# taaha-khan/2023-CompaCT-Image-Compression

Measured on AMD Instinct MI355X. Metric: MPixels/s encode+decode, 12-bit 512x512 CT batch, bytes-exact, higher is better.
Workload: dtype u16

## Files before the change

2023-compact-image-compression_amd/csrc/api.cpp:

```cpp
#include <dlfcn.h>
#include <unistd.h>
#include <zlib.h>

#include <atomic>
#include <chrono>
#include <condition_variable>
#include <functional>
#include <cstdarg>
#include <cstdio>
#include <cstdlib>
#include <cstring>
#include <map>
#include <mutex>
#include <string>
#include <thread>
#include <vector>

#include "../../include/compact_hip.h"
#include "cct_internal.h"
#include "host.h"
#include "handoff.h"

namespace cct {
bool gilbert_table(int width, int height, int32_t *out);
// ... 108 lines not shown
	}
	DecSlot(const DecSlot &) = delete;
	DecSlot &operator=(const DecSlot &) = delete;
};
constexpr int N_DEC_SLOTS = DEC_SLOTS;

struct Context {
	bool ready = false;
	pid_t pid = 0;
	int device = -1;
	hipStream_t stream = nullptr;
	int use_graph = 1;
	int deflate_fork = 1;
	int queue_ahead = 1;
	int decode_yields = 1;
	int compact_recs = 1;
	int enc_slots = 1;
	hipStream_t stream_dec = nullptr;
	std::map<std::pair<int, int>, ShapeTables> luts;
	int use_tiles = 1;
	int stream_tpg = STREAM_TPG;
	int last_path = -1;
	int runtime_bs = 0;
	int last_dec_path = -1;
	int dbg_skip = 0;
	int tuning_build = TUNING;
	int device_deflate = 1;
	int device_inflate = 1;
	int zlib_threads = 0;
	int wg_threads = 1024;
// ... 514 lines not shown
	int rc;
	void *base[DFL_REGIONS];
	for (int r = 0; r < DFL_REGIONS; r++) {
		if (dfl_region_needed(r, strategy) && (rc = E.z_ws[r].ensure(dfl_region_bytes(r, shape)))) return rc;
		base[r] = E.z_ws[r].p;
	}
	if ((rc = E.z_out.ensure((size_t)n * out_stride))) return rc;
	if ((rc = E.z_outsizes.ensure((size_t)n * 4))) return rc;
	const bool use_fork = g_ctx.deflate_fork != 0;
	if (use_fork && !E.stream_side) {
		const int crc = exclusive_section([&]() -> int { HIP_TRY(hipStreamCreateWithFlags(&E.stream_side, hipStreamNonBlocking)); return CCT_OK; });
		if (crc) return crc;
	}
	a.in = d_in; a.in_stride = in_stride; a.in_sizes = d_in_sizes;
	dfl_bind(a, base, shape);
	a.pos_mask = (g_ctx.compact_recs && mem_level == 8 && in_stride < ((size_t)1 << 22)) ? (1u << 22) - 1u : 0xFFFFFFFFu;
	const DevBuf &mr = E.z_ws[DFL_R_MATCH];
	if (dfl_uses_chains(strategy)) {
		if (E.z_mr_cleared != mr.p || E.z_mr_cleared_cap != mr.cap || E.z_gen_passes >= 16000u) {
			HIP_TRY(hipMemsetAsync(mr.p, 0, mr.cap, E.stream));
			HIP_TRY(hipMemsetAsync(E.z_ws[DFL_R_GEN].p, 0, 256, E.stream));
			E.z_mr_cleared = mr.p; E.z_mr_cleared_cap = mr.cap; E.z_gen_passes = 0;
		}
		E.z_gen_passes++;
	}
	a.out = (uint8_t *)E.z_out.p; a.out_stride = out_stride; a.out_sizes = (uint32_t *)E.z_outsizes.p;
	memcpy(a.header13, header13, 13);
	if (g_ctx.use_graph) {
		std::vector<uint8_t> key(sizeof(DeflateArgs) + 2 * sizeof(int));
		memcpy(key.data(), &a, sizeof(DeflateArgs));
// ... 1395 lines not shown
int rule_bool(int &v) { v = v ? 1 : 0; return CCT_OK; }
const Option OPTIONS[] = {
	{"zlib_threads", &Context::zlib_threads, [](int &v) { return v < 1 ? fail(CCT_E_ARG, "zlib_threads < 1") : CCT_OK; }},
	{"tile_path", &Context::use_tiles, [](int &v) {
		if (v == 3) return fail(CCT_E_ARG, "tile_path 3 (the four-kernel pipeline) has been removed");
		v = (v >= 0 && v <= 4) ? v : 1; return (int)CCT_OK; }},
	{"stream_tpg", &Context::stream_tpg, [](int &v) { v = (v == 1 || v == 2 || v == 4) ? v : STREAM_TPG; return (int)CCT_OK; }},
	{"runtime_block_size", &Context::runtime_bs, rule_bool},
	{"device_deflate", &Context::device_deflate, rule_bool},
	{"device_inflate", &Context::device_inflate, rule_bool},
	{"deflate_graph", &Context::use_graph, rule_bool},
	{"deflate_compact_records", &Context::compact_recs, rule_bool},
	{"decode_yields", &Context::decode_yields, rule_bool},
	{"queue_ahead", &Context::queue_ahead, rule_bool},
	{"deflate_fork", &Context::deflate_fork, rule_bool},
	{"encode_slots", &Context::enc_slots, [](int &v) { v = std::max(1, std::min(v, N_ENC_SLOTS)); return (int)CCT_OK; }},
	{"decode_slots", &Context::dec_slots, [](int &v) { v = std::max(1, std::min(v, N_DEC_SLOTS)); return (int)CCT_OK; }},
	{"inflate_lanes", &Context::inflate_lanes, [](int &v) {
		return v != 0 && v != 256 && v != 512 ? fail(CCT_E_ARG, "inflate_lanes must be 0 (automatic), 256 or 512") : CCT_OK; }},
	{"png_unfilter_waves", &Context::png_unfilter_waves, [](int &v) {
		return v != 1 && v != 2 && v != 4 && v != 8 ? fail(CCT_E_ARG, "png_unfilter_waves must be 1, 2, 4 or 8") : CCT_OK; }},
	{"wg_threads", &Context::wg_threads, [](int &v) {
		return v != 256 && v != 512 && v != 1024 ? fail(CCT_E_ARG, "wg_threads must be 256, 512 or 1024") : CCT_OK; }},
	{"last_encode_path", &Context::last_path, nullptr, true},
	{"last_decode_path", &Context::last_dec_path, nullptr, true},
	{"last_inflate_lanes", &Context::last_inflate_lanes, nullptr, true},
	{"debug_skip", &Context::dbg_skip, rule_any, false, true},
	{"tuning_build", &Context::tuning_build, nullptr, true, true},
};
const Option *find_option(const char *key)
// ... 31 lines not shown
```

2023-compact-image-compression_amd/csrc/deflate_kernels.hip:

```cpp
#include <hip/hip_runtime.h>
#include <cstring>
#include <algorithm>

#include "cct_internal.h"
#include "wave_device.h"
#include "../../include/compact_hip.h"

namespace cct {
namespace {

constexpr int MIN_MATCH = 3, MAX_MATCH = 258, WSIZE = 32768;
constexpr int MIN_LOOKAHEAD = MAX_MATCH + MIN_MATCH + 1;
constexpr int MAX_DIST = WSIZE - MIN_LOOKAHEAD;
constexpr int TOO_FAR = 4096;
constexpr int BLOCK_SYMS = 16383;
constexpr int BLOCK_SYMS_ML9 = 32767;
constexpr int L_CODES = 286, D_CODES = 30, BL_CODES = 19, HEAP_SIZE = 2 * L_CODES + 1;
constexpr int END_BLOCK = 256, MAX_BITS = 15, MAX_BL_BITS = 7;
constexpr uint32_t Z_FILTERED = 1, Z_HUFFMAN_ONLY = 2, Z_RLE = 3, Z_FIXED = 4;
__host__ __device__ __forceinline__ bool short_pass(uint32_t strategy) { return strategy == Z_HUFFMAN_ONLY || strategy == Z_RLE; }

__constant__ uint8_t c_extra_lbits[29] = {0,0,0,0,0,0,0,0,1,1,1,1,2,2,2,2,3,3,3,3,4,4,4,4,5,5,5,5,0};
__constant__ uint8_t c_extra_dbits[30] = {0,0,0,0,1,1,2,2,3,3,4,4,5,5,6,6,7,7,8,8,9,9,10,10,11,11,12,12,13,13};
__constant__ uint8_t c_extra_blbits[19] = {0,0,0,0,0,0,0,0,0,0,0,0,0,0,0,0,2,3,7};
// ... 988 lines not shown
	alignas(16) uint32_t heap[HEAP_SIZE + 11];
	uint32_t bl_count[MAX_BITS + 1];
	uint16_t next_code[MAX_BITS + 1];
	int heap_len, heap_max, max_code, overflow, lmax, dmax;
	uint32_t opt_len, static_len, dyn_body_bits;
	uint32_t hdr_bits[160];
	uint32_t hdr_nbits;
	int ntok, btype, max_blindex;
	uint8_t extra_l[29], extra_d[30], extra_bl[19], bl_order[19];
	__device__ __forceinline__ uint32_t *hist_l() { return heap; }
	__device__ __forceinline__ uint32_t *hist_d() { return heap + L_CODES + 2; }
	__device__ __forceinline__ uint8_t *length_code() { return reinterpret_cast<uint8_t *>(dad); }
	__device__ __forceinline__ uint8_t *dist_code() { return reinterpret_cast<uint8_t *>(dad) + 256; }
	__device__ __forceinline__ uint16_t *tok() { return dad; }
};
static_assert(sizeof(TreeScratch) <= 8192, "13 tree waves per CU: keep the working set around 8 KB");
static_assert(HEAP_SIZE >= L_CODES + D_CODES, "token list fits dad[]");
static_assert((HEAP_SIZE + 1) * 4 >= (L_CODES + 2 + D_CODES) * 4 && HEAP_SIZE * 2 >= 768, "aliases fit");
__device__ __forceinline__ uint32_t static_llen(int n) { return n <= 143 ? 8u : n <= 255 ? 9u : n <= 279 ? 7u : 8u; }

typedef __attribute__((address_space(3))) uint16_t lds_u16;
struct TreeView { lds_u16 *freq, *dad, *len, *code; };

__device__ __forceinline__ void pqdownheap(TreeScratch &S, int k, int hl)
{
	const uint32_t v = S.heap[k];
	for (int j = k << 1; j <= hl; j = k << 1) {
		const uint2 pr = *reinterpret_cast<const uint2 *>(&S.heap[j]);
		const int right = (j < hl && pr.y <= (pr.x | 1023u)) ? 1 : 0;
		const uint32_t e = right ? pr.y : pr.x;
		if (v <= (e | 1023u)) break;
// ... 2 lines not shown
	}
	S.heap[k] = v;
}

__device__ __forceinline__ TreeView view_of(TreeScratch &S, int kind)
{
	if (kind == 0) return TreeView{(lds_u16 *)S.freq, (lds_u16 *)S.dad, (lds_u16 *)S.len, (lds_u16 *)S.code};
	if (kind == 1) return TreeView{(lds_u16 *)S.dfreq, (lds_u16 *)S.ddad, (lds_u16 *)S.dlen, (lds_u16 *)S.dcode};
	return TreeView{(lds_u16 *)S.bfreq, (lds_u16 *)S.bdad, (lds_u16 *)S.blen, (lds_u16 *)S.bcode};
}
__device__ __forceinline__ int elems_of(int kind) { return kind == 0 ? L_CODES : kind == 1 ? D_CODES : BL_CODES; }

__device__ void tree_leaves(TreeScratch &S, int kind)
{
	const TreeView t = view_of(S, kind);
	const int lane = threadIdx.x, elems = elems_of(kind);
	const uint64_t lt_mask = (1ull << lane) - 1ull;
	int max_code = -1;
	uint32_t nleaf = 0;
	for (int n0 = 0; n0 < elems; n0 += 64) {
		const int n = n0 + lane;
		const uint32_t f = n < elems ? t.freq[n] : 0u;
		const uint64_t bal = __ballot(f != 0);
		if (f != 0) S.heap[1 + nleaf + (uint32_t)__popcll(bal & lt_mask)] = (f << 15) | (uint32_t)n;
		else if (n < elems) t.len[n] = 0;
		if (bal) max_code = n0 + 63 - __clzll((long long)bal);
		nleaf += (uint32_t)__popcll(bal);
	}
	if (lane == 0) { S.heap_len = (int)nleaf; S.max_code = max_code; }
}

constexpr int TREE_SIFTS = 8;
__device__ void tree_heap(TreeScratch &S, int kind)
{
	const TreeView t = view_of(S, kind);
	const int lane = threadIdx.x;
	int max_code = S.max_code, h = S.heap_len;
	while (h < 2) {
		const int node = max_code < 2 ? ++max_code : 0;
		h++;
		if (lane == 0) {
			t.freq[node] = 1; S.opt_len--;
			S.heap[h] = (1u << 15) | (uint32_t)node;
			if (kind == 0) S.static_len -= static_llen(node);
			else if (kind == 1) S.static_len -= 5;
		}
	}
	__syncthreads();
	for (int d = 31 - __clz(h >> 1); d >= 0; d--) {
		const int lo = 1 << d, hi = min((2 << d) - 1, h >> 1);
		for (int n0 = lo; n0 <= hi; n0 += 64) {
			if (n0 + lane <= hi) pqdownheap(S, n0 + lane, h);
			__builtin_amdgcn_wave_barrier();
		}
	}
	if (lane < TREE_SIFTS) {
		uint32_t v = 0, k = 1, hl = 0, w = 0;
		bool moving = false;
		const uint32_t sink = HEAP_SIZE + 3 + lane;
		auto tick = [&]() {
			const uint32_t j = k << 1;
			const uint2 pr = *reinterpret_cast<const uint2 *>(&S.heap[j]);
			const uint32_t right = (j < hl && pr.y <= (pr.x | 1023u)) ? 1u : 0u;
// ... 38 lines not shown
			if (h < 2) break;
			tick();
		}
		while (__ballot(moving)) tick();
		if (lane == 0) {
			S.heap[--hm] = en;
			S.heap_len = h; S.heap_max = hm;
			S.max_code = max_code;
		}
	}
}

__device__ void tree_depths(TreeScratch &S, int kind)
{
	const TreeView t = view_of(S, kind);
	const int lane = threadIdx.x;
	const int max_length = kind == 2 ? MAX_BL_BITS : MAX_BITS;
	const int base = kind == 0 ? 257 : 0;
	const int max_code = S.max_code, heap_max = S.heap_max;
	const uint32_t root = S.heap[heap_max];
	constexpr uint16_t UNKNOWN = 0xFFFF;
	for (int h = heap_max + 1 + lane; h < HEAP_SIZE; h += 64) t.len[S.heap[h] & 1023u] = UNKNOWN;
	if (lane == 0) t.len[root & 1023u] = 0;
	if (lane <= MAX_BITS) S.bl_count[lane] = 0;
	__syncthreads();
	for (bool again = true; again;) {
		again = false;
		for (int h0 = heap_max + 1; h0 < HEAP_SIZE; h0 += 64) {
			const int h = h0 + lane;
			bool unknown = false;
			if (h < HEAP_SIZE) {
				const int n = (int)(S.heap[h] & 1023u);
				if (t.len[n] == UNKNOWN) {
					const uint32_t ld = t.len[t.dad[n]];
					if (ld == UNKNOWN) unknown = true;
					else t.len[n] = (uint16_t)min(ld + 1u, (uint32_t)max_length);
				}
			}
			if (__ballot(unknown)) again = true;
		}
		__syncthreads();
	}
	int overflow = 0;
	for (int h0 = heap_max + 1; h0 < HEAP_SIZE; h0 += 64) {
		const int h = h0 + lane;
		const bool clamped = h < HEAP_SIZE && t.len[t.dad[S.heap[h] & 1023u]] == (uint32_t)max_length;
		overflow += (int)__popcll(__ballot(clamped));
	}
	uint32_t o = 0, st = 0;
	for (int n = lane; n <= max_code; n += 64) {
		const uint32_t f = t.freq[n];
		if (f == 0) continue;
		const uint32_t bits = t.len[n];
		atomicAdd(&S.bl_count[bits], 1u);
		uint32_t xbits = 0;
		if (n >= base) xbits = kind == 0 ? S.extra_l[n - base] : kind == 1 ? S.extra_d[n] : S.extra_bl[n];
// ... 27 lines not shown
				if ((uint32_t)t.len[m] != (uint32_t)bits) {
					S.opt_len += ((uint32_t)bits - t.len[m]) * t.freq[m];
					t.len[m] = (uint16_t)bits;
				}
				n--;
			}
		}
	}
	uint32_t code = 0;
	for (int bits = 1; bits <= MAX_BITS; bits++) { code = (code + S.bl_count[bits - 1]) << 1; S.next_code[bits] = (uint16_t)code; }
}

__device__ void tree_codes(TreeScratch &S, int kind)
{
	const TreeView t = view_of(S, kind);
	const int lane = threadIdx.x, max_code = S.max_code;
	const uint64_t lt_mask = (1ull << lane) - 1ull;
	uint32_t seen[MAX_BITS + 1];
#pragma unroll
	for (int b = 1; b <= MAX_BITS; b++) seen[b] = S.next_code[b];
	for (int n0 = 0; n0 <= max_code; n0 += 64) {
		const int n = n0 + lane;
		const int len = n <= max_code ? (int)t.len[n] : 0;
		uint32_t mine = 0;
#pragma unroll
		for (int b = 1; b <= MAX_BITS; b++) {
			const uint64_t bal = __ballot(len == b);
			if (len == b) mine = seen[b] + (uint32_t)__popcll(bal & lt_mask);
			seen[b] += (uint32_t)__popcll(bal);
		}
		if (len != 0) t.code[n] = (uint16_t)(__brev(mine) >> (32 - len));
	}
}

__device__ void scan_tree_wave(TreeScratch &S, const TreeView &t, int max_code)
{
	const int lane = threadIdx.x;
	constexpr int NCH = (L_CODES + 63) / 64;
	const int n_el = max_code + 1;
	uint32_t v[NCH];
	uint64_t startmask[NCH];
#pragma unroll
	for (int c = 0; c < NCH; c++) {
		const int n = c * 64 + lane;
		v[c] = n < n_el ? (uint32_t)t.len[n] : 0xFFFFu;
		const uint32_t before = n == 0 ? 0xFFFFFFFFu : (uint32_t)t.len[max(n - 1, 0)];
		startmask[c] = __ballot(n < n_el && v[c] != before);
	}
	uint16_t *tk = S.tok();
	uint32_t base = (uint32_t)S.ntok;
#pragma unroll
	for (int c = 0; c < NCH; c++) {
// ... 47 lines not shown
		}
		base += chunk_tok;
	}
	if (lane == 0) S.ntok = (int)base;
}

__device__ __forceinline__ void hdr_or(TreeScratch &S, uint32_t pos, uint32_t value, uint32_t n)
{
	const uint32_t w = pos >> 5, sh = pos & 31u;
	atomicOr(&S.hdr_bits[w], value << sh);
	if (sh + n > 32u) atomicOr(&S.hdr_bits[w + 1], value >> (32u - sh));
}

__device__ void send_header(TreeScratch &S)
{
	const int lane = threadIdx.x;
	const int nbl = S.max_blindex + 1;
	if (lane == 0) hdr_or(S, 0, (uint32_t)(S.lmax + 1 - 257) | ((uint32_t)(S.dmax + 1 - 1) << 5) | ((uint32_t)(nbl - 4) << 10), 14);
	if (lane < nbl) hdr_or(S, 14u + 3u * (uint32_t)lane, S.blen[S.bl_order[lane]], 3);
	uint32_t base = 14u + 3u * (uint32_t)nbl;
	const uint16_t *tk = S.tok();
	const int nt = S.ntok;
	for (int c0 = 0; c0 < nt; c0 += 64) {
		const int i = c0 + lane;
		uint32_t nbits = 0, val = 0;
		if (i < nt) {
			const uint32_t sym = tk[i] & 31u, ex = tk[i] >> 5;
			const uint32_t cl = S.blen[sym];
			nbits = cl + S.extra_bl[sym];
			val = (uint32_t)S.bcode[sym] | (ex << cl);
		}
		uint32_t chunk_bits;
		const uint32_t ex = wave_excl_scan(nbits, chunk_bits);
		if (nbits) hdr_or(S, base + ex, val, nbits);
		base += chunk_bits;
	}
	if (lane == 0) S.hdr_nbits = base;
}

constexpr int TREE_BLOCKS = 1;

__device__ __forceinline__ uint32_t window_base(uint32_t top, uint32_t L, uint32_t strategy)
{
	const uint32_t lam = strategy == Z_HUFFMAN_ONLY ? 0u : strategy == Z_RLE ? (uint32_t)MAX_MATCH : (uint32_t)MIN_LOOKAHEAD - 1u;
	const uint32_t kf = L >= 65536u ? (L - 65536u) / 32768u + 1u : 0u;
	uint32_t k = 0;
	if (top >= 65536u - lam) k = min((top - (65536u - lam)) / 32768u + 1u, kf);
	if (k == kf && 32768u * k + (uint32_t)(WSIZE + MAX_DIST) <= top && L <= top + lam) k++;
	return 32768u * k;
}
__global__ void __launch_bounds__(64) dfl_tree_kernel(DeflateArgs a)
{
	__shared__ TreeScratch S4[TREE_BLOCKS];
	const int s = blockIdx.y, m0 = blockIdx.x * TREE_BLOCKS, lane = threadIdx.x;
	const uint32_t T = a.total_syms[s];
	const uint32_t L = a.in_sizes[s];
	const uint32_t BS = a.block_syms;
	uint32_t nfull = T / BS;
	if (T % BS == 0 && nfull > 0 && !short_pass(a.strategy) && a.postloop_lit[s]) nfull--;
	const uint32_t nblocks = nfull + 1;
	BlockMeta *meta = a.block_meta + (size_t)s * a.max_blocks;
	if ((uint32_t)m0 >= nblocks) return;
	const int nb = (int)min((uint32_t)TREE_BLOCKS, nblocks - (uint32_t)m0);
	const uint32_t *bend = a.blk_end + (size_t)s * a.max_blocks;
	const bool owner = lane < nb;
#ifdef CCT_TREE_PROF
	long long tp[16]; int tpi = 0;
#define TREE_STAMP() do { if (tpi < 16) tp[tpi++] = clock64(); } while (0)
#else
#define TREE_STAMP() do {} while (0)
#endif
	TREE_STAMP();

	for (int q = 0; q < nb; q++) {
		TreeScratch &S = S4[q];
		const int m = m0 + q;
		const bool last = (uint32_t)m == nblocks - 1;
		const uint32_t first = (uint32_t)m * BS;
		const uint32_t nsym = last ? T - first : BS;
		const uint32_t *sym = a.sym + (size_t)s * a.in_stride + first;
		for (int i = lane; i < HEAP_SIZE; i += 64) { S.freq[i] = 0; S.len[i] = 0; }
		for (int i = lane; i < L_CODES + 2; i += 64) S.code[i] = 0;
		for (int i = lane; i < 2 * D_CODES + 1; i += 64) { S.dfreq[i] = 0; S.dlen[i] = 0; S.ddad[i] = 0; }
		for (int i = lane; i < D_CODES + 2; i += 64) S.dcode[i] = 0;
		for (int i = lane; i < 2 * BL_CODES + 1; i += 64) { S.bfreq[i] = 0; S.blen[i] = 0; S.bdad[i] = 0; }
		for (int i = lane; i < BL_CODES + 1; i += 64) S.bcode[i] = 0;
		uint8_t *length_code = S.length_code(), *dist_code = S.dist_code();
		{
			uint8_t dc[8], lc4[4];
#pragma unroll
			for (int k = 0; k < 8; k++) dc[k] = c_dist_code[lane + 64 * k];
#pragma unroll
			for (int k = 0; k < 4; k++) lc4[k] = c_length_code[lane + 64 * k];
			const int l29 = min(lane, 28), l30 = min(lane, 29), l19 = min(lane, 18);
			const uint8_t xl = c_extra_lbits[l29], xd = c_extra_dbits[l30], xb = c_extra_blbits[l19], bo = c_bl_order[l19];
#pragma unroll
			for (int k = 0; k < 8; k++) dist_code[lane + 64 * k] = dc[k];
#pragma unroll
			for (int k = 0; k < 4; k++) length_code[lane + 64 * k] = lc4[k];
			if (lane < 29) S.extra_l[lane] = xl;
			if (lane < 30) S.extra_d[lane] = xd;
			if (lane < 19) { S.extra_bl[lane] = xb; S.bl_order[lane] = bo; }
		}
		uint32_t *hl = S.hist_l(), *hd = S.hist_d();
		for (int i = lane; i < L_CODES; i += 64) hl[i] = 0;
		if (lane < D_CODES) hd[lane] = 0;
		__syncthreads();
		{
			const uint32_t lasts = nsym ? nsym - 1 : 0;
			uint32_t nv[16];
#pragma unroll
			for (int k = 0; k < 16; k++) nv[k] = sym[min((uint32_t)(k * 64 + lane), lasts)];
			for (uint32_t i0 = 0; i0 < nsym; i0 += 64 * 16) {
				uint32_t v[16];
#pragma unroll
				for (int k = 0; k < 16; k++) v[k] = nv[k];
#pragma unroll
				for (int k = 0; k < 16; k++) nv[k] = sym[min(i0 + 1024u + (uint32_t)(k * 64 + lane), lasts)];
#pragma unroll
				for (int k = 0; k < 16; k++) {
					if (i0 + (uint32_t)(k * 64 + lane) >= nsym) continue;
					const uint32_t dist = v[k] >> 16, lc = v[k] & 0xFFu;
					if (dist == 0) atomicAdd(&hl[lc], 1u);
					else {
						const uint32_t d1 = dist - 1;
						atomicAdd(&hl[length_code[lc] + 256 + 1], 1u);
						atomicAdd(&hd[d1 < 256 ? dist_code[d1] : dist_code[256 + (d1 >> 7)]], 1u);
					}
				}
			}
		}
		__syncthreads();
		for (int i = lane; i < L_CODES; i += 64) S.freq[i] = (uint16_t)hl[i];
		if (lane < D_CODES) S.dfreq[lane] = (uint16_t)hd[lane];
		for (int i = lane; i < 160; i += 64) S.hdr_bits[i] = 0;
		if (lane == 0) { S.opt_len = 0; S.static_len = 0; S.hdr_nbits = 0; S.ntok = 0; S.btype = 0; S.max_blindex = 0; }
		__syncthreads();
		if (lane == 0) S.freq[END_BLOCK] = 1;
		for (int i = lane; i < HEAP_SIZE; i += 64) S.dad[i] = 0;
	}
	__syncthreads();
	TREE_STAMP();
#pragma unroll 1
	for (int kind = 0; kind < 3; kind++) {
		if (kind == 2) {
			if (owner) S4[lane].dyn_body_bits = S4[lane].opt_len;
			__syncthreads();
			for (int q = 0; q < nb; q++) {
				TreeScratch &S = S4[q];
				scan_tree_wave(S, view_of(S, 0), S.lmax);
				__syncthreads();
				scan_tree_wave(S, view_of(S, 1), S.dmax);
				__syncthreads();
				if (lane < BL_CODES) { S.bfreq[lane] = (uint16_t)S.hdr_bits[lane]; S.hdr_bits[lane] = 0; }
			}
			__syncthreads();
		}
		for (int q = 0; q < nb; q++) tree_leaves(S4[q], kind);
		__syncthreads();
		TREE_STAMP();
		for (int q = 0; q < nb; q++) tree_heap(S4[q], kind);
		__syncthreads();
		TREE_STAMP();
		for (int q = 0; q < nb; q++) tree_depths(S4[q], kind);
		__syncthreads();
		if (owner) {
			tree_fix(S4[lane], kind);
			if (kind == 0) S4[lane].lmax = S4[lane].max_code; else if (kind == 1) S4[lane].dmax = S4[lane].max_code;
		}
		__syncthreads();
		for (int q = 0; q < nb; q++) tree_codes(S4[q], kind);
		__syncthreads();
		TREE_STAMP();
	}
	if (owner) {
		TreeScratch &S = S4[lane];
		const int m = m0 + lane;
		const bool last = (uint32_t)m == nblocks - 1;
		const uint32_t first = (uint32_t)m * BS;
		const uint32_t nsym = last ? T - first : BS;
		const uint32_t in_begin = m == 0 ? 0u : bend[m - 1];
		const uint32_t in_end = last ? L : bend[m];
		int max_blindex;
		for (max_blindex = BL_CODES - 1; max_blindex >= 3; max_blindex--)
			if (S.blen[S.bl_order[max_blindex]] != 0) break;
		S.opt_len += 3 * ((uint32_t)max_blindex + 1) + 5 + 5 + 4;
		uint32_t opt_lenb = (S.opt_len + 3 + 7) >> 3;
		const uint32_t static_lenb = (S.static_len + 3 + 7) >> 3;
		if (static_lenb <= opt_lenb) opt_lenb = static_lenb;
		const uint32_t stored_len = in_end - in_begin;
		const bool in_window = in_begin >= window_base(last ? L : a.blk_top[(size_t)s * a.max_blocks + m], L, a.strategy);
		BlockMeta bm;
		bm.in_begin = in_begin; bm.stored_len = stored_len; bm.first_sym = first; bm.nsym = nsym; bm.last = last ? 1u : 0u;
		if (in_window && stored_len + 4 <= opt_lenb) {
			bm.type = 0; bm.hdr_nbits = 0; bm.body_bits = 0;
		} else if (a.strategy == Z_FIXED || static_lenb == opt_lenb) {
			bm.type = 1; bm.hdr_nbits = 0; bm.body_bits = S.static_len;
		} else {
			bm.type = 2; bm.hdr_nbits = 0;
			bm.body_bits = S.dyn_body_bits;
		}
		S.btype = (int)bm.type; S.max_blindex = max_blindex;
		meta[m] = bm;
		if (m == 0) a.n_blocks[s] = nblocks;
	}
	__syncthreads();
	for (int q = 0; q < nb; q++) {
		TreeScratch &S = S4[q];
		if (S.btype != 2) continue;
		send_header(S);
		__syncthreads();
		BlockTables *bt = a.block_tables + ((size_t)s * a.max_blocks + m0 + q);
		for (int i = lane; i * 32 < (int)S.hdr_nbits; i += 64) bt->hdr_bits[i] = S.hdr_bits[i];
		if (lane == 0) meta[m0 + q].hdr_nbits = S.hdr_nbits;
	}
	__syncthreads();
	TREE_STAMP();
#ifdef CCT_TREE_PROF
	if (s == 0 && m0 == 0 && lane == 0) {
		printf("[tree prof] nb=%d:", nb);
		for (int i = 1; i < tpi; i++) printf(" %lld", tp[i] - tp[i - 1]);
		printf("  (hist | leaves0 heap0 rest0 | scan+leaves1 heap1 rest1 | scan_tree+leaves2 heap2 rest2 | final)\n");
	}
#endif
	for (int q = 0; q < nb; q++) {
		TreeScratch &S = S4[q];
		BlockTables *bt = a.block_tables + ((size_t)s * a.max_blocks + m0 + q);
		for (int i = lane; i < L_CODES; i += 64) { bt->lcode[i] = S.code[i]; bt->llen[i] = (uint8_t)S.len[i]; }
		if (lane < D_CODES) { bt->dcode[lane] = S.dcode[lane]; bt->dlen[lane] = (uint8_t)S.dlen[lane]; }
	}
}

__global__ void __launch_bounds__(256) dfl_adler_kernel(DeflateArgs a)
{
	__shared__ unsigned long long sa[256], sb[256];
	const int s = blockIdx.x;
	const uint32_t L = a.in_sizes[s];
	const uint8_t *in = a.in + (size_t)s * a.in_stride;
	unsigned long long A = 0, B = 0;
	const uint32_t nfull = L / 16;
	constexpr int U = 8;
	for (uint32_t g0 = threadIdx.x; g0 < nfull; g0 += blockDim.x * U) {
		uint4 v[U];
#pragma unroll
		for (int u = 0; u < U; u++) v[u] = *reinterpret_cast<const uint4 *>(in + (size_t)min(g0 + (uint32_t)u * blockDim.x, nfull - 1) * 16);
// ... 317 lines not shown
		return true;
	}
	if (!deflate_level_args(level, a)) return false;
	if (strategy == (int)Z_FIXED) a.zlib_flg = 0x01;
	return true;
}

bool deflate_mem_level_args(int mem_level, DeflateArgs &a)
{
	if (mem_level != 8 && mem_level != 9) return false;
	a.hash_bits = (uint32_t)mem_level + 7u;
	a.block_syms = (1u << (mem_level + 6)) - 1u;
	return true;
}

hipError_t deflate_init_tables()
{
	uint8_t length_code[256]; uint16_t base_length[29]; uint8_t dist_code[512]; uint16_t base_dist[30];
	uint16_t static_lcode[288]; uint8_t static_llen[288]; uint16_t static_dcode[30];
	static const int xl[29] = {0,0,0,0,0,0,0,0,1,1,1,1,2,2,2,2,3,3,3,3,4,4,4,4,5,5,5,5,0};
	static const int xd[30] = {0,0,0,0,1,1,2,2,3,3,4,4,5,5,6,6,7,7,8,8,9,9,10,10,11,11,12,12,13,13};
	int length = 0, code, n, dist = 0;
	for (code = 0; code < 28; code++) {
		base_length[code] = (uint16_t)length;
		for (n = 0; n < (1 << xl[code]); n++) length_code[length++] = (uint8_t)code;
	}
	length_code[length - 1] = (uint8_t)code;
	base_length[28] = 0;
	for (code = 0; code < 16; code++) {
		base_dist[code] = (uint16_t)dist;
// ... 11 lines not shown
	while (n <= 279) { static_llen[n++] = 7; bl_count[7]++; }
	while (n <= 287) { static_llen[n++] = 8; bl_count[8]++; }
	unsigned c = 0;
	for (int bits = 1; bits <= 15; bits++) { c = (c + bl_count[bits - 1]) << 1; next_code[bits] = (uint16_t)c; }
	auto rev = [](unsigned v, int len) { unsigned r = 0; do { r |= v & 1; v >>= 1; r <<= 1; } while (--len > 0); return r >> 1; };
	for (n = 0; n < 288; n++) static_lcode[n] = (uint16_t)rev(next_code[static_llen[n]]++, static_llen[n]);
	for (n = 0; n < 30; n++) static_dcode[n] = (uint16_t)rev((unsigned)n, 5);
	hipError_t e;
	if ((e = hipMemcpyToSymbol(HIP_SYMBOL(c_length_code), length_code, sizeof length_code)) != hipSuccess) return e;
	if ((e = hipMemcpyToSymbol(HIP_SYMBOL(c_base_length), base_length, sizeof base_length)) != hipSuccess) return e;
	if ((e = hipMemcpyToSymbol(HIP_SYMBOL(c_dist_code), dist_code, sizeof dist_code)) != hipSuccess) return e;
	if ((e = hipMemcpyToSymbol(HIP_SYMBOL(c_base_dist), base_dist, sizeof base_dist)) != hipSuccess) return e;
	if ((e = hipMemcpyToSymbol(HIP_SYMBOL(c_static_lcode), static_lcode, sizeof static_lcode)) != hipSuccess) return e;
	if ((e = hipMemcpyToSymbol(HIP_SYMBOL(c_static_llen), static_llen, sizeof static_llen)) != hipSuccess) return e;
	if ((e = hipMemcpyToSymbol(HIP_SYMBOL(c_static_dcode), static_dcode, sizeof static_dcode)) != hipSuccess) return e;
	return hipSuccess;
}

static hipError_t launch_deflate_short(const DeflateArgs &a, int n, hipStream_t st)
{
	const bool ml9 = a.block_syms == (uint32_t)BLOCK_SYMS_ML9;
	const int gx = (int)std::min<size_t>(64, (a.in_stride + 255) / 256);
	launch_clear(a, n, st);
	if (a.strategy == Z_RLE) {
		hipLaunchKernelGGL((dfl_run_len_kernel<false, 15>), dim3(gx, n), dim3(256), 0, st, a);
		hipLaunchKernelGGL(dfl_rle_rec_kernel, dim3(gx, n), dim3(256), 0, st, a);
		hipLaunchKernelGGL(dfl_offsets2_kernel, dim3(256), dim3(256), 0, st, a, n);
		hipLaunchKernelGGL(dfl_walk_kernel, dim3(n), dim3(WALK_T), 0, st, a, n);
		if (ml9) hipLaunchKernelGGL(dfl_symbols_kernel<BLOCK_SYMS_ML9>, dim3(gx, n), dim3(256), 0, st, a);
		else hipLaunchKernelGGL(dfl_symbols_kernel<BLOCK_SYMS>, dim3(gx, n), dim3(256), 0, st, a);
	} else {
		if (ml9) hipLaunchKernelGGL(dfl_huff_symbols_kernel<BLOCK_SYMS_ML9>, dim3(gx, n), dim3(256), 0, st, a);
		else hipLaunchKernelGGL(dfl_huff_symbols_kernel<BLOCK_SYMS>, dim3(gx, n), dim3(256), 0, st, a);
	}
	hipLaunchKernelGGL(dfl_adler_kernel, dim3(n), dim3(256), 0, st, a);
	hipLaunchKernelGGL(dfl_tree_kernel, dim3((a.max_blocks + TREE_BLOCKS - 1) / TREE_BLOCKS, n), dim3(64), 0, st, a);
	hipLaunchKernelGGL(dfl_layout_kernel, dim3(n), dim3(64), 0, st, a, n);
	hipLaunchKernelGGL(dfl_emit_kernel, dim3(a.max_blocks, n), dim3(256), 0, st, a);
	return hipGetLastError();
}

hipError_t launch_deflate(const DeflateArgs &a, int n, hipStream_t st, hipStream_t side, const hipEvent_t *ev)
{
	hipError_t e;
	const bool ml9 = a.hash_bits == 16;
	if ((a.hash_bits != 15 && !ml9) || a.block_syms != (uint32_t)(ml9 ? BLOCK_SYMS_ML9 : BLOCK_SYMS)) return hipErrorInvalidValue;
	if (ml9 && a.pos_mask != 0xFFFFFFFFu) return hipErrorInvalidValue;
	if ((a.out_stride & 3) || ((uintptr_t)a.out & 3)) return hipErrorInvalidValue;
	if (short_pass(a.strategy)) return launch_deflate_short(a, n, st);
	hipLaunchKernelGGL(dfl_offsets_kernel, dim3(64), dim3(256), 0, st, a, n);
	const int gx = (int)std::min<size_t>(64, (a.in_stride + 255) / 256);
	if (ml9) {
		hipLaunchKernelGGL((dfl_run_len_kernel<true, 16>), dim3(gx, n), dim3(256), 0, st, a);
		hipLaunchKernelGGL((dfl_sort_pass_kernel<true, 16>), dim3(n), dim3(1024), 0, st, a);
		hipLaunchKernelGGL((dfl_sort_pass_kernel<false, 16>), dim3(n), dim3(1024), 0, st, a);
	} else {
		hipLaunchKernelGGL((dfl_run_len_kernel<true, 15>), dim3(gx, n), dim3(256), 0, st, a);
		hipLaunchKernelGGL((dfl_sort_pass_kernel<true, 15>), dim3(n), dim3(1024), 0, st, a);
		hipLaunchKernelGGL((dfl_sort_pass_kernel<false, 15>), dim3(n), dim3(1024), 0, st, a);
	}
	const bool fork = side != nullptr && ev != nullptr;
	hipStream_t s2 = fork ? side : st;
	if (fork) {
// ... 21 lines not shown
		if ((e = hipEventRecord(ev[2], s2)) != hipSuccess) return e;
		if ((e = hipStreamWaitEvent(s2, ev[1], 0)) != hipSuccess) return e;
		if ((e = hipStreamWaitEvent(st, ev[2], 0)) != hipSuccess) return e;
	}
	hipLaunchKernelGGL(dfl_match_heavy_kernel, dim3(gx, n8), dim3(256), 0, s2, a, n);
	hipLaunchKernelGGL(dfl_adler_kernel, dim3(n), dim3(256), 0, s2, a);
	hipLaunchKernelGGL(dfl_match_run_kernel, dim3(gx, n8), dim3(256), 0, st, a, n);
	if (fork) {
		if ((e = hipEventRecord(ev[3], s2)) != hipSuccess) return e;
		if ((e = hipStreamWaitEvent(st, ev[3], 0)) != hipSuccess) return e;
	}
	hipLaunchKernelGGL(dfl_rec_kernel, dim3(gx, n), dim3(256), 0, st, a);
	hipLaunchKernelGGL(dfl_walk_kernel, dim3(n), dim3(WALK_T), 0, st, a, n);
	if (ml9) hipLaunchKernelGGL(dfl_symbols_kernel<BLOCK_SYMS_ML9>, dim3(gx, n), dim3(256), 0, st, a);
	else hipLaunchKernelGGL(dfl_symbols_kernel<BLOCK_SYMS>, dim3(gx, n), dim3(256), 0, st, a);
	hipLaunchKernelGGL(dfl_tree_kernel, dim3((a.max_blocks + TREE_BLOCKS - 1) / TREE_BLOCKS, n), dim3(64), 0, st, a);
	hipLaunchKernelGGL(dfl_layout_kernel, dim3(n), dim3(64), 0, st, a, n);
	hipLaunchKernelGGL(dfl_emit_kernel, dim3(a.max_blocks, n), dim3(256), 0, st, a);
	return hipGetLastError();
}

__global__ void __launch_bounds__(256) dfl_pack_exact_kernel(const uint8_t *src, size_t stride, const uint32_t *sizes,
                                                             const uint64_t *offsets, uint8_t *dst)
{
	const int s = blockIdx.y;
	const uint32_t nbytes = sizes[s];
	const uint8_t *in = src + (size_t)s * stride;
	uint8_t *out = dst + offsets[s];
	const uint32_t head = min((uint32_t)(-(uintptr_t)out & 3u), nbytes);
	const uint32_t nd = (nbytes - head) >> 2;
	const uint32_t tid = blockIdx.x * blockDim.x + threadIdx.x, nth = gridDim.x * blockDim.x;
// ... 23 lines not shown
```

2023-compact-image-compression_amd/csrc/deflate_workspace.h:

```cpp
#pragma once
#include <stddef.h>
#include <stdint.h>

#if defined(__HIPCC__)
#include <hip/hip_runtime.h>
#define DFL_HD __host__ __device__ __forceinline__
#else
#define DFL_HD inline
#endif

namespace cct {

struct BlockMeta {
	uint64_t bit_off;
	uint32_t type;
	uint32_t last;
	uint32_t first_sym, nsym;
	uint32_t in_begin, stored_len;
	uint32_t hdr_nbits, body_bits;
};
struct BlockTables {
	uint16_t lcode[286]; uint8_t llen[286];
	uint16_t dcode[30]; uint8_t dlen[30];
	uint32_t hdr_bits[160];
// ... 9 lines not shown
	uint32_t *run_counts; int run_chunks;
	uint32_t *sort_hist;
	uint16_t *run_len;
	uint32_t *rec32, *exit_pos, *exit_cnt;
	uint32_t *blk_entry, *blk_symbase;
	uint32_t *total_syms, *postloop_lit, *n_blocks, *adler, *heavy_count, *deep_count, *run_end_count;
	uint32_t *blk_end;
	uint32_t *blk_top;
	BlockMeta *block_meta; BlockTables *block_tables;
	int max_blocks;
	uint8_t *out; size_t out_stride; uint32_t *out_sizes;
	uint8_t header13[16];
	uint32_t good, max_lazy, nice, max_chain, zlib_flg;
	uint32_t strategy, min_len;
	uint32_t hash_bits, block_syms;
};

constexpr int SORT_HIST = 512;
constexpr int RUNLEN_OUT = 2048 - 264;
constexpr int BLK_ENTRY_GRAIN = 64;
enum DflCounter { DFL_SEG_BEGIN, DFL_SEG_END, DFL_TOTAL_SYMS, DFL_POSTLOOP_LIT, DFL_N_BLOCKS, DFL_ADLER, DFL_HEAVY_COUNT,
                  DFL_DEEP_COUNT, DFL_RUN_END_COUNT, DFL_COUNTERS };

DFL_HD int dfl_run_chunks(size_t in_stride) { return (int)(in_stride / RUNLEN_OUT + 1); }
DFL_HD int dfl_max_blocks(size_t in_stride, uint32_t block_syms) { return (int)(in_stride / block_syms + 2); }
DFL_HD size_t dfl_blk_words(size_t in_stride) { return in_stride / BLK_ENTRY_GRAIN; }
DFL_HD size_t dfl_hist_words(size_t n, size_t run_chunks) { return n * (SORT_HIST + 2 * run_chunks); }

DFL_HD size_t zlib_bound(size_t n, bool mem_level_8)
{
// ... 85 lines not shown
```

Baseline: 17960.

## Pack sixteen Huffman tree waves per workgroup with device-side launch selection

The deflate tree kernel now runs one deflate block per wavefront and can pack 16 waves per workgroup, each with its own LDS TreeScratch. Workgroup barriers become wavefront-scoped fences and barriers. In automatic mode both the 16-wave and 1-wave variants are launched, and each decides on the device, from the total workgroup count versus the CU count, whether it should do the work. This is meant to spread tree building across more CUs and raise occupancy, at the cost of an extra kernel launch and a per-wave scan over all slices' block counts.

```diff
diff --git a/2023-compact-image-compression_amd/csrc/api.cpp b/2023-compact-image-compression_amd/csrc/api.cpp
--- a/2023-compact-image-compression_amd/csrc/api.cpp
+++ b/2023-compact-image-compression_amd/csrc/api.cpp
@@ -146,6 +146,7 @@
 	int deflate_fork = 1;
 	int queue_ahead = 1;
 	int decode_yields = 1;
+	int tree_waves = 0;
 	int compact_recs = 1;
 	int enc_slots = 1;
 	hipStream_t stream_dec = nullptr;
@@ -690,6 +691,7 @@
 	}
 	a.in = d_in; a.in_stride = in_stride; a.in_sizes = d_in_sizes;
 	dfl_bind(a, base, shape);
+	a.tree_waves = (uint32_t)g_ctx.tree_waves;
 	a.pos_mask = (g_ctx.compact_recs && mem_level == 8 && in_stride < ((size_t)1 << 22)) ? (1u << 22) - 1u : 0xFFFFFFFFu;
 	const DevBuf &mr = E.z_ws[DFL_R_MATCH];
 	if (dfl_uses_chains(strategy)) {
@@ -2115,6 +2117,8 @@
 	{"decode_yields", &Context::decode_yields, rule_bool},
 	{"queue_ahead", &Context::queue_ahead, rule_bool},
 	{"deflate_fork", &Context::deflate_fork, rule_bool},
+	{"tree_waves", &Context::tree_waves, [](int &v) {
+		return v != 0 && v != 1 && v != 16 ? fail(CCT_E_ARG, "tree_waves must be 0 (automatic), 1 or 16") : CCT_OK; }},
 	{"encode_slots", &Context::enc_slots, [](int &v) { v = std::max(1, std::min(v, N_ENC_SLOTS)); return (int)CCT_OK; }},
 	{"decode_slots", &Context::dec_slots, [](int &v) { v = std::max(1, std::min(v, N_DEC_SLOTS)); return (int)CCT_OK; }},
 	{"inflate_lanes", &Context::inflate_lanes, [](int &v) {
diff --git a/2023-compact-image-compression_amd/csrc/deflate_kernels.hip b/2023-compact-image-compression_amd/csrc/deflate_kernels.hip
--- a/2023-compact-image-compression_amd/csrc/deflate_kernels.hip
+++ b/2023-compact-image-compression_amd/csrc/deflate_kernels.hip
@@ -1026,7 +1026,12 @@
 	__device__ __forceinline__ uint8_t *dist_code() { return reinterpret_cast<uint8_t *>(dad) + 256; }
 	__device__ __forceinline__ uint16_t *tok() { return dad; }
 };
-static_assert(sizeof(TreeScratch) <= 8192, "13 tree waves per CU: keep the working set around 8 KB");
+static_assert(16 * sizeof(TreeScratch) <= 160 * 1024, "a workgroup of 16 tree waves has to fit the LDS of a CU");
+__device__ __forceinline__ void tree_wave_sync()
+{
+	__builtin_amdgcn_fence(__ATOMIC_ACQ_REL, "wavefront");
+	__builtin_amdgcn_wave_barrier();
+}
 static_assert(HEAP_SIZE >= L_CODES + D_CODES, "token list fits dad[]");
 static_assert((HEAP_SIZE + 1) * 4 >= (L_CODES + 2 + D_CODES) * 4 && HEAP_SIZE * 2 >= 768, "aliases fit");
 __device__ __forceinline__ uint32_t static_llen(int n) { return n <= 143 ? 8u : n <= 255 ? 9u : n <= 279 ? 7u : 8u; }
@@ -1059,7 +1064,7 @@
 __device__ void tree_leaves(TreeScratch &S, int kind)
 {
 	const TreeView t = view_of(S, kind);
-	const int lane = threadIdx.x, elems = elems_of(kind);
+	const int lane = threadIdx.x & 63, elems = elems_of(kind);
 	const uint64_t lt_mask = (1ull << lane) - 1ull;
 	int max_code = -1;
 	uint32_t nleaf = 0;
@@ -1079,7 +1084,7 @@
 __device__ void tree_heap(TreeScratch &S, int kind)
 {
 	const TreeView t = view_of(S, kind);
-	const int lane = threadIdx.x;
+	const int lane = threadIdx.x & 63;
 	int max_code = S.max_code, h = S.heap_len;
 	while (h < 2) {
 		const int node = max_code < 2 ? ++max_code : 0;
@@ -1091,7 +1096,7 @@
 			else if (kind == 1) S.static_len -= 5;
 		}
 	}
-	__syncthreads();
+	tree_wave_sync();
 	for (int d = 31 - __clz(h >> 1); d >= 0; d--) {
 		const int lo = 1 << d, hi = min((2 << d) - 1, h >> 1);
 		for (int n0 = lo; n0 <= hi; n0 += 64) {
@@ -1160,7 +1165,7 @@
 __device__ void tree_depths(TreeScratch &S, int kind)
 {
 	const TreeView t = view_of(S, kind);
-	const int lane = threadIdx.x;
+	const int lane = threadIdx.x & 63;
 	const int max_length = kind == 2 ? MAX_BL_BITS : MAX_BITS;
 	const int base = kind == 0 ? 257 : 0;
 	const int max_code = S.max_code, heap_max = S.heap_max;
@@ -1169,7 +1174,7 @@
 	for (int h = heap_max + 1 + lane; h < HEAP_SIZE; h += 64) t.len[S.heap[h] & 1023u] = UNKNOWN;
 	if (lane == 0) t.len[root & 1023u] = 0;
 	if (lane <= MAX_BITS) S.bl_count[lane] = 0;
-	__syncthreads();
+	tree_wave_sync();
 	for (bool again = true; again;) {
 		again = false;
 		for (int h0 = heap_max + 1; h0 < HEAP_SIZE; h0 += 64) {
@@ -1185,7 +1190,7 @@
 			}
 			if (__ballot(unknown)) again = true;
 		}
-		__syncthreads();
+		tree_wave_sync();
 	}
 	int overflow = 0;
 	for (int h0 = heap_max + 1; h0 < HEAP_SIZE; h0 += 64) {
@@ -1243,7 +1248,7 @@
 __device__ void tree_codes(TreeScratch &S, int kind)
 {
 	const TreeView t = view_of(S, kind);
-	const int lane = threadIdx.x, max_code = S.max_code;
+	const int lane = threadIdx.x & 63, max_code = S.max_code;
 	const uint64_t lt_mask = (1ull << lane) - 1ull;
 	uint32_t seen[MAX_BITS + 1];
 #pragma unroll
@@ -1264,7 +1269,7 @@
 
 __device__ void scan_tree_wave(TreeScratch &S, const TreeView &t, int max_code)
 {
-	const int lane = threadIdx.x;
+	const int lane = threadIdx.x & 63;
 	constexpr int NCH = (L_CODES + 63) / 64;
 	const int n_el = max_code + 1;
 	uint32_t v[NCH];
@@ -1342,7 +1347,7 @@
 
 __device__ void send_header(TreeScratch &S)
 {
-	const int lane = threadIdx.x;
+	const int lane = threadIdx.x & 63;
 	const int nbl = S.max_blindex + 1;
 	if (lane == 0) hdr_or(S, 0, (uint32_t)(S.lmax + 1 - 257) | ((uint32_t)(S.dmax + 1 - 1) << 5) | ((uint32_t)(nbl - 4) << 10), 14);
 	if (lane < nbl) hdr_or(S, 14u + 3u * (uint32_t)lane, S.blen[S.bl_order[lane]], 3);
@@ -1366,8 +1371,6 @@
 	if (lane == 0) S.hdr_nbits = base;
 }
 
-constexpr int TREE_BLOCKS = 1;
-
 __device__ __forceinline__ uint32_t window_base(uint32_t top, uint32_t L, uint32_t strategy)
 {
 	const uint32_t lam = strategy == Z_HUFFMAN_ONLY ? 0u : strategy == Z_RLE ? (uint32_t)MAX_MATCH : (uint32_t)MIN_LOOKAHEAD - 1u;
@@ -1377,21 +1380,63 @@
 	if (k == kf && 32768u * k + (uint32_t)(WSIZE + MAX_DIST) <= top && L <= top + lam) k++;
 	return 32768u * k;
 }
-__global__ void __launch_bounds__(64) dfl_tree_kernel(DeflateArgs a)
-{
-	__shared__ TreeScratch S4[TREE_BLOCKS];
-	const int s = blockIdx.y, m0 = blockIdx.x * TREE_BLOCKS, lane = threadIdx.x;
+#ifdef CCT_TREE_PROF
+struct TreeProbe { uint32_t hw_id, xcc_id, slice, block; uint64_t rt0, rt1, cycles; };
+constexpr int TREE_PROBE_CAP = 16384;
+__device__ TreeProbe g_tree_probe[TREE_PROBE_CAP];
+extern "C" int cct_tree_prof_reset()
+{
+	void *p;
+	if (hipGetSymbolAddress(&p, HIP_SYMBOL(g_tree_probe)) != hipSuccess) return -1;
+	return hipMemset(p, 0, sizeof(TreeProbe) * TREE_PROBE_CAP) == hipSuccess && hipDeviceSynchronize() == hipSuccess ? 0 : -1;
+}
+extern "C" int cct_tree_prof_read(void *out, int cap)
+{
+	const int n = cap < TREE_PROBE_CAP ? cap : TREE_PROBE_CAP;
+	if (hipDeviceSynchronize() != hipSuccess) return -1;
+	return hipMemcpyFromSymbol(out, HIP_SYMBOL(g_tree_probe), sizeof(TreeProbe) * (size_t)n) == hipSuccess ? n : -1;
+}
+#define TREE_PROBE_ENTER() const uint64_t prt0 = __builtin_amdgcn_s_memrealtime(), pmt0 = __builtin_amdgcn_s_memtime()
+#define TREE_PROBE_EXIT(s_, m_, max_blocks_) do { \
+		const uint64_t pmt1 = __builtin_amdgcn_s_memtime(), prt1 = __builtin_amdgcn_s_memrealtime(); \
+		const uint32_t pidx = (uint32_t)(s_) * (uint32_t)(max_blocks_) + (uint32_t)(m_); \
+		if (lane == 0 && pidx < (uint32_t)TREE_PROBE_CAP) \
+			g_tree_probe[pidx] = TreeProbe{(uint32_t)__builtin_amdgcn_s_getreg(4 | (31 << 11)) , \
+			                               (uint32_t)__builtin_amdgcn_s_getreg(20 | (31 << 11)) , \
+			                               (uint32_t)(s_), (uint32_t)(m_), prt0, prt1, pmt1 - pmt0}; \
+	} while (0)
+#else
+#define TREE_PROBE_ENTER() do {} while (0)
+#define TREE_PROBE_EXIT(s_, m_, max_blocks_) do {} while (0)
+#endif
+__device__ __forceinline__ uint32_t tree_nblocks(const DeflateArgs &a, int s)
+{
+	const uint32_t T = a.total_syms[s], BS = a.block_syms;
+	uint32_t nfull = T / BS;
+	if (T % BS == 0 && nfull > 0 && !short_pass(a.strategy) && a.postloop_lit[s]) nfull--;
+	return nfull + 1;
+}
+template <int WAVES>
+__global__ void __launch_bounds__(64 * WAVES) dfl_tree_kernel(DeflateArgs a, uint32_t cus)
+{
+	extern __shared__ __attribute__((aligned(16))) uint8_t tree_lds[];
+	const int wave = WAVES == 1 ? 0 : __builtin_amdgcn_readfirstlane((int)(threadIdx.x >> 6));
+	const int s = blockIdx.x, n = gridDim.x, m = blockIdx.y * WAVES + wave, lane = threadIdx.x & 63;
+	TreeScratch &S = reinterpret_cast<TreeScratch *>(tree_lds)[wave];
 	const uint32_t T = a.total_syms[s];
 	const uint32_t L = a.in_sizes[s];
 	const uint32_t BS = a.block_syms;
-	uint32_t nfull = T / BS;
-	if (T % BS == 0 && nfull > 0 && !short_pass(a.strategy) && a.postloop_lit[s]) nfull--;
-	const uint32_t nblocks = nfull + 1;
+	const uint32_t nblocks = tree_nblocks(a, s);
 	BlockMeta *meta = a.block_meta + (size_t)s * a.max_blocks;
-	if ((uint32_t)m0 >= nblocks) return;
-	const int nb = (int)min((uint32_t)TREE_BLOCKS, nblocks - (uint32_t)m0);
+	if ((uint32_t)m >= nblocks) return;
+	if (a.tree_waves == 0) {
+		uint32_t wgs = 0;
+		for (int i = lane; i < n; i += 64) wgs += (tree_nblocks(a, i) + 15u) / 16u;
+		wgs = (uint32_t)__builtin_amdgcn_readfirstlane((int)wave_sum(wgs));
+		if ((wgs <= cus ? 16 : 1) != WAVES) return;
+	}
 	const uint32_t *bend = a.blk_end + (size_t)s * a.max_blocks;
-	const bool owner = lane < nb;
+	TREE_PROBE_ENTER();
 #ifdef CCT_TREE_PROF
 	long long tp[16]; int tpi = 0;
 #define TREE_STAMP() do { if (tpi < 16) tp[tpi++] = clock64(); } while (0)
@@ -1400,12 +1445,10 @@
 #endif
 	TREE_STAMP();
 
-	for (int q = 0; q < nb; q++) {
-		TreeScratch &S = S4[q];
-		const int m = m0 + q;
-		const bool last = (uint32_t)m == nblocks - 1;
-		const uint32_t first = (uint32_t)m * BS;
-		const uint32_t nsym = last ? T - first : BS;
+	const bool last = (uint32_t)m == nblocks - 1;
+	const uint32_t first = (uint32_t)m * BS;
+	const uint32_t nsym = last ? T - first : BS;
+	{
 		const uint32_t *sym = a.sym + (size_t)s * a.in_stride + first;
 		for (int i = lane; i < HEAP_SIZE; i += 64) { S.freq[i] = 0; S.len[i] = 0; }
 		for (int i = lane; i < L_CODES + 2; i += 64) S.code[i] = 0;
@@ -1433,7 +1476,7 @@
 		uint32_t *hl = S.hist_l(), *hd = S.hist_d();
 		for (int i = lane; i < L_CODES; i += 64) hl[i] = 0;
 		if (lane < D_CODES) hd[lane] = 0;
-		__syncthreads();
+		tree_wave_sync();
 		{
 			const uint32_t lasts = nsym ? nsym - 1 : 0;
 			uint32_t nv[16];
@@ -1458,55 +1501,47 @@
 				}
 			}
 		}
-		__syncthreads();
+		tree_wave_sync();
 		for (int i = lane; i < L_CODES; i += 64) S.freq[i] = (uint16_t)hl[i];
 		if (lane < D_CODES) S.dfreq[lane] = (uint16_t)hd[lane];
 		for (int i = lane; i < 160; i += 64) S.hdr_bits[i] = 0;
 		if (lane == 0) { S.opt_len = 0; S.static_len = 0; S.hdr_nbits = 0; S.ntok = 0; S.btype = 0; S.max_blindex = 0; }
-		__syncthreads();
+		tree_wave_sync();
 		if (lane == 0) S.freq[END_BLOCK] = 1;
 		for (int i = lane; i < HEAP_SIZE; i += 64) S.dad[i] = 0;
 	}
-	__syncthreads();
+	tree_wave_sync();
 	TREE_STAMP();
 #pragma unroll 1
 	for (int kind = 0; kind < 3; kind++) {
 		if (kind == 2) {
-			if (owner) S4[lane].dyn_body_bits = S4[lane].opt_len;
-			__syncthreads();
-			for (int q = 0; q < nb; q++) {
-				TreeScratch &S = S4[q];
-				scan_tree_wave(S, view_of(S, 0), S.lmax);
-				__syncthreads();
-				scan_tree_wave(S, view_of(S, 1), S.dmax);
-				__syncthreads();
-				if (lane < BL_CODES) { S.bfreq[lane] = (uint16_t)S.hdr_bits[lane]; S.hdr_bits[lane] = 0; }
-			}
-			__syncthreads();
-		}
-		for (int q = 0; q < nb; q++) tree_leaves(S4[q], kind);
-		__syncthreads();
+			if (lane == 0) S.dyn_body_bits = S.opt_len;
+			tree_wave_sync();
+			scan_tree_wave(S, view_of(S, 0), S.lmax);
+			tree_wave_sync();
+			scan_tree_wave(S, view_of(S, 1), S.dmax);
+			tree_wave_sync();
+			if (lane < BL_CODES) { S.bfreq[lane] = (uint16_t)S.hdr_bits[lane]; S.hdr_bits[lane] = 0; }
+			tree_wave_sync();
+		}
+		tree_leaves(S, kind);
+		tree_wave_sync();
 		TREE_STAMP();
-		for (int q = 0; q < nb; q++) tree_heap(S4[q], kind);
-		__syncthreads();
+		tree_heap(S, kind);
+		tree_wave_sync();
 		TREE_STAMP();
-		for (int q = 0; q < nb; q++) tree_depths(S4[q], kind);
-		__syncthreads();
-		if (owner) {
-			tree_fix(S4[lane], kind);
-			if (kind == 0) S4[lane].lmax = S4[lane].max_code; else if (kind == 1) S4[lane].dmax = S4[lane].max_code;
-		}
-		__syncthreads();
-		for (int q = 0; q < nb; q++) tree_codes(S4[q], kind);
-		__syncthreads();
+		tree_depths(S, kind);
+		tree_wave_sync();
+		if (lane == 0) {
+			tree_fix(S, kind);
+			if (kind == 0) S.lmax = S.max_code; else if (kind == 1) S.dmax = S.max_code;
+		}
+		tree_wave_sync();
+		tree_codes(S, kind);
+		tree_wave_sync();
 		TREE_STAMP();
 	}
-	if (owner) {
-		TreeScratch &S = S4[lane];
-		const int m = m0 + lane;
-		const bool last = (uint32_t)m == nblocks - 1;
-		const uint32_t first = (uint32_t)m * BS;
-		const uint32_t nsym = last ? T - first : BS;
+	if (lane == 0) {
 		const uint32_t in_begin = m == 0 ? 0u : bend[m - 1];
 		const uint32_t in_end = last ? L : bend[m];
 		int max_blindex;
@@ -1532,31 +1567,26 @@
 		meta[m] = bm;
 		if (m == 0) a.n_blocks[s] = nblocks;
 	}
-	__syncthreads();
-	for (int q = 0; q < nb; q++) {
-		TreeScratch &S = S4[q];
-		if (S.btype != 2) continue;
+	tree_wave_sync();
+	BlockTables *bt = a.block_tables + ((size_t)s * a.max_blocks + m);
+	if (S.btype == 2) {
 		send_header(S);
-		__syncthreads();
-		BlockTables *bt = a.block_tables + ((size_t)s * a.max_blocks + m0 + q);
+		tree_wave_sync();
 		for (int i = lane; i * 32 < (int)S.hdr_nbits; i += 64) bt->hdr_bits[i] = S.hdr_bits[i];
-		if (lane == 0) meta[m0 + q].hdr_nbits = S.hdr_nbits;
-	}
-	__syncthreads();
+		if (lane == 0) meta[m].hdr_nbits = S.hdr_nbits;
+	}
+	tree_wave_sync();
 	TREE_STAMP();
 #ifdef CCT_TREE_PROF
-	if (s == 0 && m0 == 0 && lane == 0) {
-		printf("[tree prof] nb=%d:", nb);
+	if (s == 0 && m == 0 && lane == 0) {
+		printf("[tree prof] waves=%d:", WAVES);
 		for (int i = 1; i < tpi; i++) printf(" %lld", tp[i] - tp[i - 1]);
 		printf("  (hist | leaves0 heap0 rest0 | scan+leaves1 heap1 rest1 | scan_tree+leaves2 heap2 rest2 | final)\n");
 	}
 #endif
-	for (int q = 0; q < nb; q++) {
-		TreeScratch &S = S4[q];
-		BlockTables *bt = a.block_tables + ((size_t)s * a.max_blocks + m0 + q);
-		for (int i = lane; i < L_CODES; i += 64) { bt->lcode[i] = S.code[i]; bt->llen[i] = (uint8_t)S.len[i]; }
-		if (lane < D_CODES) { bt->dcode[lane] = S.dcode[lane]; bt->dlen[lane] = (uint8_t)S.dlen[lane]; }
-	}
+	for (int i = lane; i < L_CODES; i += 64) { bt->lcode[i] = S.code[i]; bt->llen[i] = (uint8_t)S.len[i]; }
+	if (lane < D_CODES) { bt->dcode[lane] = S.dcode[lane]; bt->dlen[lane] = (uint8_t)S.dlen[lane]; }
+	TREE_PROBE_EXIT(s, m, a.max_blocks);
 }
 
 __global__ void __launch_bounds__(256) dfl_adler_kernel(DeflateArgs a)
@@ -1904,6 +1934,7 @@
 	return true;
 }
 
+static int g_tree_cus = 0;
 hipError_t deflate_init_tables()
 {
 	uint8_t length_code[256]; uint16_t base_length[29]; uint8_t dist_code[512]; uint16_t base_dist[30];
@@ -1945,7 +1976,26 @@
 	if ((e = hipMemcpyToSymbol(HIP_SYMBOL(c_static_lcode), static_lcode, sizeof static_lcode)) != hipSuccess) return e;
 	if ((e = hipMemcpyToSymbol(HIP_SYMBOL(c_static_llen), static_llen, sizeof static_llen)) != hipSuccess) return e;
 	if ((e = hipMemcpyToSymbol(HIP_SYMBOL(c_static_dcode), static_dcode, sizeof static_dcode)) != hipSuccess) return e;
-	return hipSuccess;
+	int dev;
+	if ((e = hipGetDevice(&dev)) != hipSuccess) return e;
+	if ((e = hipDeviceGetAttribute(&g_tree_cus, hipDeviceAttributeMultiprocessorCount, dev)) != hipSuccess) return e;
+	return hipFuncSetAttribute(reinterpret_cast<const void *>(dfl_tree_kernel<16>), hipFuncAttributeMaxDynamicSharedMemorySize,
+	                           (int)(16 * sizeof(TreeScratch)));
+}
+
+constexpr int TREE_WAVES16_MIN_SLICES = 128;
+template <int WAVES>
+static void launch_tree_waves(const DeflateArgs &a, int n, hipStream_t st)
+{
+	hipLaunchKernelGGL(dfl_tree_kernel<WAVES>, dim3(n, (a.max_blocks + WAVES - 1) / WAVES), dim3(64 * WAVES),
+	                   WAVES * sizeof(TreeScratch), st, a, (uint32_t)g_tree_cus);
+}
+static void launch_tree(const DeflateArgs &a0, int n, hipStream_t st)
+{
+	DeflateArgs a = a0;
+	if (a.tree_waves == 0 && (n < TREE_WAVES16_MIN_SLICES || n > g_tree_cus)) a.tree_waves = 1;
+	if (a.tree_waves != 1) launch_tree_waves<16>(a, n, st);
+	if (a.tree_waves != 16) launch_tree_waves<1>(a, n, st);
 }
 
 static hipError_t launch_deflate_short(const DeflateArgs &a, int n, hipStream_t st)
@@ -1965,7 +2015,7 @@
 		else hipLaunchKernelGGL(dfl_huff_symbols_kernel<BLOCK_SYMS>, dim3(gx, n), dim3(256), 0, st, a);
 	}
 	hipLaunchKernelGGL(dfl_adler_kernel, dim3(n), dim3(256), 0, st, a);
-	hipLaunchKernelGGL(dfl_tree_kernel, dim3((a.max_blocks + TREE_BLOCKS - 1) / TREE_BLOCKS, n), dim3(64), 0, st, a);
+	launch_tree(a, n, st);
 	hipLaunchKernelGGL(dfl_layout_kernel, dim3(n), dim3(64), 0, st, a, n);
 	hipLaunchKernelGGL(dfl_emit_kernel, dim3(a.max_blocks, n), dim3(256), 0, st, a);
 	return hipGetLastError();
@@ -1978,6 +2028,7 @@
 	if ((a.hash_bits != 15 && !ml9) || a.block_syms != (uint32_t)(ml9 ? BLOCK_SYMS_ML9 : BLOCK_SYMS)) return hipErrorInvalidValue;
 	if (ml9 && a.pos_mask != 0xFFFFFFFFu) return hipErrorInvalidValue;
 	if ((a.out_stride & 3) || ((uintptr_t)a.out & 3)) return hipErrorInvalidValue;
+	if (a.tree_waves != 0 && a.tree_waves != 1 && a.tree_waves != 16) return hipErrorInvalidValue;
 	if (short_pass(a.strategy)) return launch_deflate_short(a, n, st);
 	hipLaunchKernelGGL(dfl_offsets_kernel, dim3(64), dim3(256), 0, st, a, n);
 	const int gx = (int)std::min<size_t>(64, (a.in_stride + 255) / 256);
@@ -2029,7 +2080,7 @@
 	hipLaunchKernelGGL(dfl_walk_kernel, dim3(n), dim3(WALK_T), 0, st, a, n);
 	if (ml9) hipLaunchKernelGGL(dfl_symbols_kernel<BLOCK_SYMS_ML9>, dim3(gx, n), dim3(256), 0, st, a);
 	else hipLaunchKernelGGL(dfl_symbols_kernel<BLOCK_SYMS>, dim3(gx, n), dim3(256), 0, st, a);
-	hipLaunchKernelGGL(dfl_tree_kernel, dim3((a.max_blocks + TREE_BLOCKS - 1) / TREE_BLOCKS, n), dim3(64), 0, st, a);
+	launch_tree(a, n, st);
 	hipLaunchKernelGGL(dfl_layout_kernel, dim3(n), dim3(64), 0, st, a, n);
 	hipLaunchKernelGGL(dfl_emit_kernel, dim3(a.max_blocks, n), dim3(256), 0, st, a);
 	return hipGetLastError();
diff --git a/2023-compact-image-compression_amd/csrc/deflate_workspace.h b/2023-compact-image-compression_amd/csrc/deflate_workspace.h
--- a/2023-compact-image-compression_amd/csrc/deflate_workspace.h
+++ b/2023-compact-image-compression_amd/csrc/deflate_workspace.h
@@ -47,6 +47,7 @@
 	uint32_t good, max_lazy, nice, max_chain, zlib_flg;
 	uint32_t strategy, min_len;
 	uint32_t hash_bits, block_syms;
+	uint32_t tree_waves;
 };
 
 constexpr int SORT_HIST = 512;
```

New measurement: 18330 (median of 6 runs). 1.02x the previous value.
